# leimao/Voice-Converter-CycleGAN

Measured on NVIDIA H100. Metric: CycleGAN-VC train steps/sec @ batch 256x[24,128] MCEP, higher is better.
Workload: dtype f16f8 (forward / data gradient: fp16 MMA + two e4m3 cross-term MMAs = 2 MMA units per product; weight gradient: fp16 MMA alone, 1 unit; f32 accumulate)

## Files before the change

### voice-converter-cyclegan_b200/csrc/geom.h

```cpp
#pragma once
#include "kernels.cuh"
#include <string.h>
#include <vector>

static inline void same_pad(int n, int k, int s, int& before, int& out) {
  out = (n + s - 1) / s;
  int total = (out - 1) * s + k - n; if (total < 0) total = 0;
  before = total / 2;
}

static inline GatherGeom fwd_geom(int B, int H, int W, int kh, int kw, int sh, int sw) {
  GatherGeom g; memset(&g, 0, sizeof g);
  int ph, pw, Ho, Wo; same_pad(H, kh, sh, ph, Ho); same_pad(W, kw, sw, pw, Wo);
  g.B = B; g.Hy = Ho; g.Wx = Wo; g.Hs = H; g.Ws = W; g.sy = sh; g.sx = sw;
  g.Hd = Ho; g.Wd = Wo; g.dsy = 1; g.dsx = 1; g.doy = 0; g.dox = 0;
  g.ntaps = 0;
  for (int i = 0; i < kh; ++i) for (int j = 0; j < kw; ++j) {
    g.oy[g.ntaps] = (short)(i - ph); g.ox[g.ntaps] = (short)(j - pw); g.widx[g.ntaps] = (short)(i * kw + j); g.ntaps++;
  }
  return g;
}

static inline bool divisible(int v, int s) { return ((v % s) + s) % s == 0; }

static inline std::vector<GatherGeom> dgrad_geoms(int B, int H, int W, int kh, int kw, int sh, int sw) {
  std::vector<GatherGeom> out;
  int ph, pw, Ho, Wo; same_pad(H, kh, sh, ph, Ho); same_pad(W, kw, sw, pw, Wo);
  for (int py = 0; py < sh; ++py) for (int px = 0; px < sw; ++px) {
    GatherGeom g; memset(&g, 0, sizeof g);
    g.B = B; g.Hy = (H - py + sh - 1) / sh; g.Wx = (W - px + sw - 1) / sw;
    if (g.Hy <= 0 || g.Wx <= 0) continue;
    g.Hs = Ho; g.Ws = Wo; g.sy = 1; g.sx = 1;
    g.Hd = H; g.Wd = W; g.dsy = sh; g.dsx = sw; g.doy = py; g.dox = px;
    g.ntaps = 0;
    for (int i = 0; i < kh; ++i) for (int j = 0; j < kw; ++j) {
      if (!divisible(py + ph - i, sh) || !divisible(px + pw - j, sw)) continue;
      g.oy[g.ntaps] = (short)((py + ph - i) / sh); g.ox[g.ntaps] = (short)((px + pw - j) / sw);
      g.widx[g.ntaps] = (short)(i * kw + j); g.ntaps++;
    }
    out.push_back(g);
  }
  return out;
}
```

### voice-converter-cyclegan_b200/csrc/kernels.cuh

```cuda
#pragma once
#include <cuda_runtime.h>
#include <cuda_bf16.h>
#include <cuda_fp16.h>
#include <cuda_fp8.h>
#include <stdint.h>

#define CGVC_Q_ACT_SHI 1.0f
#define CGVC_Q_ACT_SLO 4096.0f
#define CGVC_Q_W_SHI 8.0f
#define CGVC_Q_W_SLO 32768.0f
#define CGVC_Q_ACC_SHIFT 15
#ifdef __CUDACC__
__device__ __forceinline__ uint32_t cgvc_e4m3x4(float a, float b, float c, float d) {
  const uint32_t lo = (uint32_t)__nv_cvt_float2_to_fp8x2(make_float2(a, b), __NV_SATFINITE, __NV_E4M3);
  const uint32_t hi = (uint32_t)__nv_cvt_float2_to_fp8x2(make_float2(c, d), __NV_SATFINITE, __NV_E4M3);
  return lo | (hi << 16);
}
__device__ __forceinline__ void cgvc_quant4(const float (&v)[4], float s_hi, float s_lo, uint2& q16, uint32_t& q8hi, uint32_t& q8lo) {
  const __half2 h01 = __floats2half2_rn(v[0], v[1]), h23 = __floats2half2_rn(v[2], v[3]);
  const float2 f01 = __half22float2(h01), f23 = __half22float2(h23);
  q16.x = *reinterpret_cast<const uint32_t*>(&h01); q16.y = *reinterpret_cast<const uint32_t*>(&h23);
  q8hi = cgvc_e4m3x4(f01.x * s_hi, f01.y * s_hi, f23.x * s_hi, f23.y * s_hi);
  q8lo = cgvc_e4m3x4((v[0] - f01.x) * s_lo, (v[1] - f01.y) * s_lo, (v[2] - f23.x) * s_lo, (v[3] - f23.y) * s_lo);
}
#endif

extern unsigned long long g_cgvc_launches;

#define CGVC_NUM_SMS 132

#define CGVC_MAX_TAPS 18

struct GatherGeom {
  int B, Hy, Wx;
  int Hs, Ws;
  int sy, sx;
  int ntaps;
  int Hd, Wd, dsy, dsx, doy, dox;
  short oy[CGVC_MAX_TAPS], ox[CGVC_MAX_TAPS], widx[CGVC_MAX_TAPS];
};

struct PackGeom { const long long* off; int n; int div; int max_len; };
#ifdef __CUDACC__
__device__ __forceinline__ int pack_find(const long long* __restrict__ off, int n, long long f) {
  int lo = 0, hi = n;
  while (hi - lo > 1) { const int mid = (lo + hi) >> 1; if (__ldg(off + mid) <= f) lo = mid; else hi = mid; }
  return lo;
}
#endif

struct GemmOperands {
  const float* src; int s_ld; int s_coff; int C;
  const float* w; long long w_ts; int w_cs; int w_ns;
  int N;
  float* dst; int d_ld; int d_coff;
  const float* bias;
  int accumulate;
};

cudaError_t launch_gg_simt(const GatherGeom& g, const GemmOperands& op, cudaStream_t st);
cudaError_t launch_gg_simt_packed(const GatherGeom& g, const GemmOperands& op, const PackGeom& pk, cudaStream_t st);
cudaError_t launch_wgrad_simt(const GatherGeom& g, const float* src, int s_ld, int s_coff, int C,
                              const float* grad, int g_ld, int g_coff, int N,
                              float* dw, long long w_ts, int w_cs, int w_ns, cudaStream_t st);
cudaError_t launch_colsum(const float* grad, long long rows, int g_ld, int g_coff, int N, float* db, cudaStream_t st);

struct PostParams {
  const float* p; int ldp; int Cc;
  int B, R, C, sh;
  const float *beta_a, *gamma_a, *beta_g, *gamma_g;
  int has_in, has_gate;
  const float* resid;
  float* y;
  float* stats;
  __nv_bfloat16 *y_hi, *y_lo;
  float* scratch;
  int qmode;
  PackGeom seg; long long seg_rows;
};
cudaError_t launch_post_fwd(const PostParams& pp, cudaStream_t st);

struct PostBwdParams {
  const float* dy1; const float* dy2;
  const float* p; int ldp; int Cc;
// ... 62 lines not shown
```

### voice-converter-cyclegan_b200/csrc/tc_gemm.cu

```cuda
#include "tc_gemm.cuh"
#include "geom.h"
#include "kernels.cuh"
#include "wgmma.cuh"

#include <cuda.h>
#include <stdint.h>
#include <stdio.h>

namespace {

typedef CUresult (*EncodeTiledFn)(CUtensorMap*, CUtensorMapDataType, cuuint32_t, void*, const cuuint64_t*, const cuuint64_t*,
                                  const cuuint32_t*, const cuuint32_t*, CUtensorMapInterleave, CUtensorMapSwizzle,
                                  CUtensorMapL2promotion, CUtensorMapFloatOOBfill);
EncodeTiledFn get_encoder() {
  static EncodeTiledFn fn = nullptr;
  if (!fn) {
    void* p = nullptr; cudaDriverEntryPointQueryResult q;
    if (cudaGetDriverEntryPoint("cuTensorMapEncodeTiled", &p, cudaEnableDefault, &q) == cudaSuccess && q == cudaDriverEntryPointSuccess)
      fn = (EncodeTiledFn)p;
  }
  return fn;
}
bool make_tmap3(CUtensorMap* m, const void* base, uint64_t d0, uint64_t d1, uint64_t d2, uint32_t b1) {
  EncodeTiledFn enc = get_encoder();
// ... 65 lines not shown
__device__ __forceinline__ void mbar_arrive(uint64_t* bar) {
  asm volatile("mbarrier.arrive.shared::cta.b64 _, [%0];" ::"r"(smem_u32(bar)) : "memory");
}
__device__ __forceinline__ void consumer_bar() { asm volatile("bar.sync 3, 256;" ::: "memory"); }
__device__ __forceinline__ void st_shared16(uint32_t addr, uint4 v) {
  asm volatile("st.shared.v4.b32 [%0], {%1, %2, %3, %4};" ::"r"(addr), "r"(v.x), "r"(v.y), "r"(v.z), "r"(v.w) : "memory");
}
__device__ __forceinline__ uint4 e4m3x8_to_f16x8(uint2 v) {
  uint32_t w[4];
#pragma unroll
  for (int i = 0; i < 4; ++i) {
    const uint32_t src = (i < 2 ? v.x : v.y) >> (16 * (i & 1));
    const __half2_raw h = __nv_cvt_fp8x2_to_halfraw2((__nv_fp8x2_storage_t)(src & 0xFFFFu), __NV_E4M3);
    w[i] = (uint32_t)h.x | ((uint32_t)h.y << 16);
  }
  return make_uint4(w[0], w[1], w[2], w[3]);
}

struct FastDiv { uint32_t mul, shr, d; };
__host__ inline FastDiv make_fastdiv(uint32_t d) {
  FastDiv f; f.d = d;
  uint32_t l = 0; while ((1ull << l) < d) ++l;
  f.mul = (uint32_t)(((1ull << 32) * ((1ull << l) - d)) / d + 1);
  f.shr = l;
  return f;
}
__device__ __forceinline__ uint32_t fdiv(uint32_t n, const FastDiv& f) { return (uint32_t)(((uint64_t)__umulhi(n, f.mul) + n) >> f.shr); }

__device__ __forceinline__ uint32_t sw128(int r, int c) { return (uint32_t)((r >> 3) * 1024 + (r & 7) * 128 + ((c ^ (r & 7)) << 4)); }

struct TcNTParams {
  GatherGeom g;
  const __nv_bfloat16 *a_hi, *a_lo; int a_ld; int C;
  const __nv_bfloat16 *b_hi, *b_lo; int Nw;
  int N;
  int n_tiles;
  int debug;
  float* dst; int d_ld; const float* bias; int accumulate;
  int perm; int Cc;
  int R;
  const float *gamma_a, *beta_a, *gamma_g, *beta_g;
  float* stats;
  const float* resid;
  float* y; __nv_bfloat16 *y_hi, *y_lo;
  int C_out;
  const float* bp; int bp_ld;
  __nv_bfloat16 *dp_hi, *dp_lo; int dp_ld;
  float *dbeta_a, *dgamma_a, *dbeta_g, *dgamma_g;
  CUtensorMap tm_b_hi, tm_b_lo;
  const uint8_t *a8_hi, *a8_lo;
  CUtensorMap tm_b8_hi, tm_b8_lo;
  uint8_t* y8;
  PackGeom pk;
};

struct TcTNParams {
  GatherGeom g;
  const __nv_bfloat16 *x_hi, *x_lo; int x_ld; int C;
  const __nv_bfloat16 *g_hi, *g_lo; int g_ld; int N;
  float* dw_a; float* dw_g; int n_split;
  int ksplit;
  FastDiv div_hw, div_w;
  CUtensorMap tm_g_hi, tm_g_lo;
  const uint8_t *x8_hi, *x8_lo;
  const uint8_t *g8_hi, *g8_lo;
  int w16;
  int fold_n;
};

__device__ __forceinline__ float* tn_dst(float* base, int slab, int C, int c, int ncols, int col, int fold_n) {
  if (fold_n) { const int t = col / fold_n; return base + ((long long)t * C + c) * fold_n + (col - t * fold_n); }
  return base + ((long long)slab * C + c) * ncols + col;
}

constexpr int kProducerThreads = 128;


template <int BN, int NPL>
struct NTCfg {
  static constexpr int A_PLANE = 128 * 128;
  static constexpr int B_PLANE = BN * 128;
  static constexpr int PLANES = NPL == 2 ? 2 : 1;
  static constexpr int STAGE = PLANES * (A_PLANE + B_PLANE);
  static constexpr int STAGES = (192 * 1024) / STAGE;
  static constexpr int SMEM = STAGES * STAGE + 1024;
  static_assert(STAGES * STAGE >= 128 * BN * 4, "the finished fp32 tile is staged over the pipeline stages");
};

template <int BN>
__device__ __forceinline__ int acc_off(int r, int n) { return r * BN + (n & ~31) + ((((n >> 2) & 7) ^ (r & 7)) << 2) + (n & 3); }
template <int BN>
__device__ __forceinline__ void acc_ld32(const float* acc, int r, int col, uint32_t (&v)[32]) {
#pragma unroll
  for (int c = 0; c < 8; ++c) {
    const float4 x = *reinterpret_cast<const float4*>(acc + r * BN + col + ((c ^ (r & 7)) << 2));
    v[4 * c] = __float_as_uint(x.x); v[4 * c + 1] = __float_as_uint(x.y); v[4 * c + 2] = __float_as_uint(x.z); v[4 * c + 3] = __float_as_uint(x.w);
  }
}

__device__ __forceinline__ float warp_colsum32(float (&t)[32], int lane) {
#pragma unroll
  for (int o = 16, n = 32; o >= 1; o >>= 1, n >>= 1) {
    const bool up = (lane & o) != 0;
#pragma unroll
    for (int i = 0; i < n / 2; ++i) {
      float send = up ? t[i] : t[i + n / 2];
      float keep = up ? t[i + n / 2] : t[i];
      t[i] = keep + __shfl_xor_sync(0xffffffffu, send, o);
    }
  }
  return t[0];
}
__device__ __forceinline__ void epi_bar(int id) { asm volatile("bar.sync %0, 128;" ::"r"(id) : "memory"); }

__device__ __forceinline__ float sample_sum(float v, float (*xch)[32], int q, int lane, int spw, int barid) {
  if (spw == 1) return v;
  epi_bar(barid);
  xch[q][lane] = v;
  epi_bar(barid);
  const int q0 = (q / spw) * spw;
  float r = 0.f;
  for (int w = 0; w < spw; ++w) r += xch[q0 + w][lane];
  return r;
}
__device__ __forceinline__ void bc4(const float* p, float (&v)[4]) { const float4 x = *reinterpret_cast<const float4*>(p); v[0] = x.x; v[1] = x.y; v[2] = x.z; v[3] = x.w; }
__device__ __forceinline__ float fast_sigmoid(float x) { return __fdividef(1.f, 1.f + __expf(-x)); }
__device__ __forceinline__ void chunk_norm_coeffs(const float (&v)[32], const float* __restrict__ gamma, const float* __restrict__ beta,
                                                  int ch, int R, float (*xch)[32], float* bc, int q, int lane, int spw, int barid, float& mean, float& rstd) {
  float t[32];
// ... 111 lines not shown
    rows_out(stg, y, lane, [&](int rr, int w0, float4 val) {
      if (mq + rr < M) *reinterpret_cast<float4*>(yf + ((mq + rr) * rs + ro) * C + ch + w0) = val;
    });
  float hl[32];
#pragma unroll
  for (int k = 0; k < 16; ++k) {
    __nv_bfloat162 hh = __floats2bfloat162_rn(y[2 * k], y[2 * k + 1]);
    float2 f = __bfloat1622float2(hh);
    __nv_bfloat162 ll = __floats2bfloat162_rn(y[2 * k] - f.x, y[2 * k + 1] - f.y);
    hl[k] = __uint_as_float(*reinterpret_cast<uint32_t*>(&hh)); hl[16 + k] = __uint_as_float(*reinterpret_cast<uint32_t*>(&ll));
  }
  rows_out(stg, hl, lane, [&](int rr, int w0, float4 val) {
    __nv_bfloat16* plane = (w0 < 16) ? yhi : ylo;
    if (mq + rr < M) *reinterpret_cast<float4*>(plane + ((mq + rr) * rs + ro) * C + ch + 2 * (w0 & 15)) = val;
  });
}
__device__ __forceinline__ void hwrite_yq(float* stg, const float (&y)[32], float* yf, __nv_bfloat16* q16, uint8_t* q8,
                                          long long mq, long long M, int C, int ch, int lane, int rs = 1, int ro = 0) {
  if (yf)
    rows_out(stg, y, lane, [&](int rr, int w0, float4 val) {
      if (mq + rr < M) *reinterpret_cast<float4*>(yf + ((mq + rr) * rs + ro) * C + ch + w0) = val;
    });
  float w[32];
#pragma unroll
  for (int k = 0; k < 8; ++k) {
    const float v[4] = {y[4 * k], y[4 * k + 1], y[4 * k + 2], y[4 * k + 3]};
    uint2 h; uint32_t b_hi, b_lo;
    cgvc_quant4(v, CGVC_Q_ACT_SHI, CGVC_Q_ACT_SLO, h, b_hi, b_lo);
    w[2 * k] = __uint_as_float(h.x); w[2 * k + 1] = __uint_as_float(h.y);
    w[16 + k] = __uint_as_float(b_hi); w[24 + k] = __uint_as_float(b_lo);
  }
  rows_out(stg, w, lane, [&](int rr, int w0, float4 val) {
    if (mq + rr >= M) return;
    const long long r = (mq + rr) * rs + ro;
    uint8_t* dst;
    if (w0 < 16) dst = reinterpret_cast<uint8_t*>(q16) + (r * C + ch + 2 * w0) * 2;
    else if (w0 < 24) dst = q8 + r * C + ch + 4 * (w0 - 16);
    else dst = q8 + M * rs * C + r * C + ch + 4 * (w0 - 24);
    *reinterpret_cast<float4*>(dst) = val;
  });
}

template <int BN, int NPL, int EPI>
__device__ __forceinline__ void nt_tile_epilogue(const TcNTParams& p, const long long M, const int HW, const long long m0, const int n0,
                                                 const int q, const int lane, float* stg, float** rowp, float* bc, float (*epi_xch)[32],
                                                 const float* acc, const int grp = 0, const int ngrp = 1) {
  const GatherGeom& g = p.g;
  const int barid = 1 + grp;
  const int arow = q * 32 + lane;
  const long long mq = m0 + q * 32;
  const long long m = mq + lane;
  float* drow = nullptr;
  if (m < M && p.dst) {
    int b = (int)(m / HW); int rem = (int)(m - (long long)b * HW);
    int y = rem / g.Wx; int x = rem - y * g.Wx;
    long long dr = ((long long)(b * g.Hd + y * g.dsy + g.doy) * g.Wd + x * g.dsx + g.dox);
    drow = p.dst + dr * p.d_ld;
  }
  __syncwarp();
  rowp[lane] = drow;
  __syncwarp();
  {
    const int spw = p.R >> 5;
    const long long sample = mq / p.R;
    const bool stat_writer = (q % spw) == 0 && mq < M && p.stats != nullptr;
    if (EPI == 1) {
      const int ch0 = n0 >> 1;
#pragma unroll 1
      for (int cb = grp; cb < 4; cb += ngrp) {
        const int ch = ch0 + cb * 32;
        float va[32], vg[32];
        { uint32_t u[32]; acc_ld32<BN>(acc, arow, (cb * 32), u);
#pragma unroll
          for (int k = 0; k < 32; k += 4) { float4 bb = *reinterpret_cast<const float4*>(p.bias + n0 + cb * 32 + k);
            va[k] = __uint_as_float(u[k]) + bb.x; va[k + 1] = __uint_as_float(u[k + 1]) + bb.y; va[k + 2] = __uint_as_float(u[k + 2]) + bb.z; va[k + 3] = __uint_as_float(u[k + 3]) + bb.w; } }
        { uint32_t u[32]; acc_ld32<BN>(acc, arow, (128 + cb * 32), u);
#pragma unroll
          for (int k = 0; k < 32; k += 4) { float4 bb = *reinterpret_cast<const float4*>(p.bias + n0 + 128 + cb * 32 + k);
            vg[k] = __uint_as_float(u[k]) + bb.x; vg[k + 1] = __uint_as_float(u[k + 1]) + bb.y; vg[k + 2] = __uint_as_float(u[k + 2]) + bb.z; vg[k + 3] = __uint_as_float(u[k + 3]) + bb.w; } }
        if (p.dst) {
          hwrite_rows_f32(stg, va, rowp, ch, lane);
          hwrite_rows_f32(stg, vg, rowp, p.Cc + ch, lane);
        }
        float mean_a, rstd_a, mean_g, rstd_g;
        chunk_norm_coeffs(va, p.gamma_a, p.beta_a, ch, p.R, epi_xch, bc, q, lane, spw, barid, mean_a, rstd_a);
        chunk_norm_coeffs(vg, p.gamma_g, p.beta_g, ch, p.R, epi_xch, bc + 64, q, lane, spw, barid, mean_g, rstd_g);
        if (stat_writer) {
          float* st = p.stats + sample * 4 * p.C_out + ch + lane;
          st[0] = mean_a; st[p.C_out] = rstd_a; st[2 * p.C_out] = mean_g; st[3 * p.C_out] = rstd_g;
        }
#pragma unroll
        for (int k = 0; k < 32; k += 4) {
          float4 sa = *reinterpret_cast<const float4*>(bc + k), oa = *reinterpret_cast<const float4*>(bc + 32 + k);
          float4 sg = *reinterpret_cast<const float4*>(bc + 64 + k), og = *reinterpret_cast<const float4*>(bc + 96 + k);
          va[k]     = fmaf(va[k],     sa.x, oa.x) * fast_sigmoid(fmaf(vg[k],     sg.x, og.x));
          va[k + 1] = fmaf(va[k + 1], sa.y, oa.y) * fast_sigmoid(fmaf(vg[k + 1], sg.y, og.y));
          va[k + 2] = fmaf(va[k + 2], sa.z, oa.z) * fast_sigmoid(fmaf(vg[k + 2], sg.z, og.z));
          va[k + 3] = fmaf(va[k + 3], sa.w, oa.w) * fast_sigmoid(fmaf(vg[k + 3], sg.w, og.w));
        }
        if (NPL == 3) hwrite_yq(stg, va, p.y, p.y_hi, p.y8, mq, M, p.C_out, ch, lane);
        else hwrite_y(stg, va, p.y, p.y_hi, p.y_lo, mq, M, p.C_out, ch, lane);
      }
    } else if (EPI == 5) {
      const int Ch = p.C_out;
      const int ch0 = n0 >> 2;
#pragma unroll 1
      for (int cb = grp; cb < 2; cb += ngrp) {
        const int ch = ch0 + cb * 32;
// ... 202 lines not shown
          wgmma_e4m3<BN>(d, make_desc(sA + 64 + k * 32, 16, 1024), make_desc64(sB + k * 32), 1);
        }
      } else if constexpr (KIND == MMA_F16) {
#pragma unroll
        for (int k = 0; k < 4; ++k)
          wgmma_f16<BN, 0, 0>(d, make_desc(sA + k * 32, 16, 1024), make_desc(sB + k * 32, 16, 1024), 1);
      } else {
#pragma unroll
        for (int k = 0; k < 4; ++k) {
          const uint64_t a_hi = make_desc(sA + k * 32, 16, 1024), b_hi = make_desc(sB + k * 32, 16, 1024);
          wgmma_bf16<BN, 0, 0>(d, a_hi, b_hi, 1);
          if constexpr (KIND == MMA_BF16X3) {
            const uint64_t a_lo = make_desc(sA + Cfg::A_PLANE + k * 32, 16, 1024), b_lo = make_desc(sB + Cfg::B_PLANE + k * 32, 16, 1024);
            wgmma_bf16<BN, 0, 0>(d, a_hi, b_lo, 1);
            wgmma_bf16<BN, 0, 0>(d, a_lo, b_hi, 1);
          }
        }
      }
    } else {
#pragma unroll
      for (int k = 0; k < 4; ++k) {
        const uint64_t a0 = make_desc(sA + k * 2048, 8192, 1024), b0 = make_desc(sB + k * 2048, 8192, 1024);
        const uint64_t a1 = make_desc(sA + Cfg::A_PLANE + k * 2048, 8192, 1024), b1 = make_desc(sB + Cfg::B_PLANE + k * 2048, 8192, 1024);
        if constexpr (KIND == MMA_F16_CROSS) {
          wgmma_f16<BN, 1, 1>(d, a0, b1, 1);
          wgmma_f16<BN, 1, 1>(d, a1, b0, 1);
        } else if constexpr (KIND == MMA_F16) {
          wgmma_f16<BN, 1, 1>(d, a0, b0, 1);
        } else {
          wgmma_bf16<BN, 1, 1>(d, a0, b0, 1);
          if constexpr (KIND == MMA_BF16X3) {
            wgmma_bf16<BN, 1, 1>(d, a0, b1, 1);
            wgmma_bf16<BN, 1, 1>(d, a1, b0, 1);
          }
        }
      }
    }
    wgmma_commit();
    wgmma_wait<1>();
    fence_acc(d);
    if (prev >= 0 && lane == 0) mbar_arrive(&empty_bar[prev]);
    prev = stage;
    if (++stage == Cfg::STAGES) { stage = 0; phase ^= 1; }
  }
}
template <int N>
__device__ __forceinline__ void rescale_acc(float (&d)[N], float scale) {
  wgmma_wait<0>();
  fence_acc(d);
#pragma unroll
  for (int i = 0; i < N; ++i) d[i] *= scale;
}

template <int BN>
__device__ __forceinline__ void nt_store_fragments(const TcNTParams& p, const float (&d)[BN / 2], const long long M, const int HW,
                                                   const long long m0, const int n0, const int r, const int c) {
  const GatherGeom& g = p.g;
  float* rowp[2];
#pragma unroll
  for (int h = 0; h < 2; ++h) {
    const long long m = m0 + r + 8 * h;
    rowp[h] = nullptr;
    if (m < M && p.dst) {
      int b = (int)(m / HW); int rem = (int)(m - (long long)b * HW);
      int y = rem / g.Wx; int x = rem - y * g.Wx;
      rowp[h] = p.dst + ((long long)(b * g.Hd + y * g.dsy + g.doy) * g.Wd + x * g.dsx + g.dox) * p.d_ld;
    }
  }
  const bool vec = (p.d_ld & 1) == 0;
#pragma unroll
  for (int j = 0; j < BN / 8; ++j) {
    const int cb = j >> 2;
    const int n = (p.perm == 2 ? (cb >> 2) * p.Cc + ((cb >> 1) & 1) * (p.Cc >> 1) + (n0 >> 2) + (cb & 1) * 32
                   : p.perm    ? ((cb < 4) ? (n0 >> 1) + cb * 32 : p.Cc + (n0 >> 1) + (cb - 4) * 32) : n0 + cb * 32) + ((8 * j) & 31) + c;
    if (n >= p.N) continue;
    float2 bb = make_float2(0.f, 0.f);
    if (p.bias) bb = *reinterpret_cast<const float2*>(p.bias + n0 + 8 * j + c);
#pragma unroll
    for (int h = 0; h < 2; ++h) {
      float* rp = rowp[h];
      if (rp == nullptr) continue;
      float v0 = d[4 * j + 2 * h], v1 = d[4 * j + 2 * h + 1];
      if (p.bias) { v0 += bb.x; v1 += bb.y; }
      if (vec && n + 2 <= p.N) {
        if (p.accumulate)
          asm volatile("red.global.add.v2.f32 [%0], {%1, %2};" ::"l"(rp + n), "f"(v0), "f"(v1) : "memory");
        else
          *reinterpret_cast<float2*>(rp + n) = make_float2(v0, v1);
      } else {
        if (p.accumulate) atomicAdd(rp + n, v0); else rp[n] = v0;
        if (n + 1 < p.N) { if (p.accumulate) atomicAdd(rp + n + 1, v1); else rp[n + 1] = v1; }
      }
    }
  }
}

constexpr int kNTThreads = 384;

template <int BN, int NPL, int EPI, bool PK = false>
__global__ void __launch_bounds__(kNTThreads, 1)
tc_gg_nt_kernel(const __grid_constant__ TcNTParams p) {
  static_assert(!PK || EPI == 0, "packed rows never take the fused epilogues (they need whole equal-length samples per tile)");
  using Cfg = NTCfg<BN, NPL>;
  __shared__ float epi_xch[2][4][32];
  __shared__ __align__(16) float epi_bc[8][(EPI == 3 || EPI == 4) ? 384 : 128];
  __shared__ __align__(16) float epi_stage[8][32 * 16];
  __shared__ float* epi_rowp[8][32];
  constexpr int S = Cfg::STAGES;
  extern __shared__ uint8_t smem_raw[];
  __shared__ __align__(8) uint64_t full_bar[S], empty_bar[S], acc_free_bar;

  const uint32_t smem_base = (smem_u32(smem_raw) + 1023u) & ~1023u;
  const int warp = threadIdx.x >> 5, lane = threadIdx.x & 31;
  const GatherGeom& g = p.g;
  const long long M = (long long)g.B * g.Hy * g.Wx;
  const int HW = g.Hy * g.Wx;
  const int cchunks = p.C >> 6;
  const int kb_pass = g.ntaps * cchunks;
  const int num_kb = NPL == 3 ? 2 * kb_pass : kb_pass;
  const int m_tiles = (int)((M + 127) / 128);
  const int n_tiles = p.n_tiles;
  const int num_tiles = m_tiles * n_tiles;

  if (threadIdx.x == 0) {
    for (int s = 0; s < S; ++s) { mbar_init(&full_bar[s], kProducerThreads + 1); mbar_init(&empty_bar[s], 8); }
    mbar_init(&acc_free_bar, 8);
    fence_barrier_init();
    tma_prefetch_desc(&p.tm_b_hi);
    if (NPL == 2) tma_prefetch_desc(&p.tm_b_lo);
    if (NPL == 3) { tma_prefetch_desc(&p.tm_b8_hi); tma_prefetch_desc(&p.tm_b8_lo); }
  }
  __syncthreads();

  if (warp < 4) {
    const int t = threadIdx.x;
    const int chunk = t & 7, rsub = t >> 3;
    int stage = 0; uint32_t phase = 0;
    int it = 0;
    for (int tile = blockIdx.x; tile < num_tiles; tile += gridDim.x, ++it) {
      const long long m0 = (long long)(tile % m_tiles) * 128;
      const int n0 = (tile / m_tiles) * BN;
      if (EPI != 0 && it > 0) mbar_wait(&acc_free_bar, (uint32_t)(it - 1) & 1u);
      int rb[8], ry[8], rx[8];
#pragma unroll
      for (int i = 0; i < 8; ++i) {
        long long m = m0 + rsub + 16 * i;
        if (m < M) {
          if constexpr (PK) {
            const int dout = p.pk.div * g.sx;
            const int u = pack_find(p.pk.off, p.pk.n, m * dout);
            const long long o0 = __ldg(p.pk.off + u), o1 = __ldg(p.pk.off + u + 1);
            rb[i] = (int)(o0 / p.pk.div); ry[i] = (int)((o1 - o0) / p.pk.div); rx[i] = (int)(m - o0 / dout) * g.sx;
          } else {
            int b = (int)(m / HW); int rem = (int)(m - (long long)b * HW);
            int y = rem / g.Wx; int x = rem - y * g.Wx;
            rb[i] = b; ry[i] = y * g.sy; rx[i] = x * g.sx;
          }
        } else { rb[i] = -1; ry[i] = 0; rx[i] = 0; }
      }
      for (int pass = 0; pass < (NPL == 3 ? 2 : 1); ++pass)
      for (int tap = 0; tap < g.ntaps; ++tap) {
        long long aoff[8];
#pragma unroll
        for (int i = 0; i < 8; ++i) {
          const int cofs = NPL == 3 && pass == 0 ? (chunk & 3) * 16 : chunk * 8;
          if constexpr (PK) {
            const int xx = rx[i] + g.ox[tap];
            aoff[i] = rb[i] >= 0 && xx >= 0 && xx < ry[i] ? (long long)(rb[i] + xx) * p.a_ld + cofs : -1;
          } else {
            int yy = ry[i] + g.oy[tap], xx = rx[i] + g.ox[tap];
            bool ok = rb[i] >= 0 && yy >= 0 && yy < g.Hs && xx >= 0 && xx < g.Ws;
            aoff[i] = ok ? ((long long)(rb[i] * g.Hs + yy) * g.Ws + xx) * p.a_ld + cofs : -1;
          }
        }
        for (int cc = 0; cc < cchunks; ++cc) {
          const int c0 = cc << 6;
          mbar_wait(&empty_bar[stage], phase ^ 1);
          const uint32_t sA = smem_base + stage * Cfg::STAGE;
          const uint32_t sB = sA + Cfg::PLANES * Cfg::A_PLANE;
          if (t == 0) {
            mbar_expect_tx(&full_bar[stage], Cfg::PLANES * Cfg::B_PLANE);
            if (NPL == 3) {
              if (pass == 0) {
                tma_load3(sB, &p.tm_b8_hi, c0, n0, g.widx[tap], &full_bar[stage]);
                tma_load3(sB + Cfg::B_PLANE / 2, &p.tm_b8_lo, c0, n0, g.widx[tap], &full_bar[stage]);
              } else {
                tma_load3(sB, &p.tm_b_hi, c0, n0, g.widx[tap], &full_bar[stage]);
              }
            } else {
              tma_load3(sB, &p.tm_b_hi, c0, n0, g.widx[tap], &full_bar[stage]);
              if (NPL == 2) tma_load3(sB + Cfg::B_PLANE, &p.tm_b_lo, c0, n0, g.widx[tap], &full_bar[stage]);
            }
          }
          if (!(p.debug & 4)) {
#pragma unroll
            for (int i = 0; i < 8; ++i) {
              const int r = rsub + 16 * i;
              const uint32_t so = sw128(r, chunk);
              const bool ok = aoff[i] >= 0;
              const long long off = ok ? aoff[i] + c0 : 0;
              if (NPL == 3) {
                if (pass == 0)
                  cp_async16(sA + so, (chunk < 4 ? p.a8_hi : p.a8_lo) + off, ok ? 16u : 0u);
                else
                  cp_async16(sA + so, p.a_hi + off, ok ? 16u : 0u);
              } else {
                cp_async16(sA + so, p.a_hi + off, ok ? 16u : 0u);
                if (NPL == 2) cp_async16(sA + Cfg::A_PLANE + so, p.a_lo + off, ok ? 16u : 0u);
              }
            }
          }
          cp_async_arrive_noinc(&full_bar[stage]);
          if (++stage == S) { stage = 0; phase ^= 1; }
        }
      }
    }
  } else {
    const int cw = warp - 4;
    const int wg = cw >> 2;
    const int tw = threadIdx.x - 128 * (wg + 1);
    float* acc_s = reinterpret_cast<float*>(smem_raw + (smem_base - smem_u32(smem_raw)));
    int stage = 0; uint32_t phase = 0;
    for (int tile = blockIdx.x; tile < num_tiles; tile += gridDim.x) {
      const long long m0 = (long long)(tile % m_tiles) * 128;
      const int n0 = (tile / m_tiles) * BN;
      float d[BN / 2];
#pragma unroll
      for (int i = 0; i < BN / 2; ++i) d[i] = 0.f;
      int prev = -1;
      if constexpr (NPL == 3) {
        consume_stages<BN, MMA_E4M3_CROSS, 0, Cfg>(d, kb_pass, stage, phase, prev, full_bar, empty_bar, smem_base, wg, lane);
        rescale_acc(d, 1.f / (float)(1 << CGVC_Q_ACC_SHIFT));
        consume_stages<BN, MMA_F16, 0, Cfg>(d, kb_pass, stage, phase, prev, full_bar, empty_bar, smem_base, wg, lane);
      } else {
        consume_stages<BN, NPL == 2 ? MMA_BF16X3 : MMA_BF16, 0, Cfg>(d, num_kb, stage, phase, prev, full_bar, empty_bar, smem_base, wg, lane);
      }
      wgmma_wait<0>();
      fence_acc(d);
      if (lane == 0) mbar_arrive(&empty_bar[prev]);
      const int r0 = wg * 64 + (tw >> 5) * 16 + ((tw & 31) >> 2), c0 = 2 * (tw & 3);
      if constexpr (EPI == 0) {
        if (!(p.debug & 3)) nt_store_fragments<BN>(p, d, M, HW, m0, n0, r0, c0);
      } else {
        consumer_bar();
        if (!(p.debug & 2)) {
#pragma unroll
          for (int j = 0; j < BN / 8; ++j) {
            *reinterpret_cast<float2*>(acc_s + acc_off<BN>(r0, 8 * j + c0)) = make_float2(d[4 * j], d[4 * j + 1]);
            *reinterpret_cast<float2*>(acc_s + acc_off<BN>(r0 + 8, 8 * j + c0)) = make_float2(d[4 * j + 2], d[4 * j + 3]);
          }
        }
        consumer_bar();
        nt_tile_epilogue<BN, NPL, EPI>(p, M, HW, m0, n0, cw & 3, lane, epi_stage[cw], epi_rowp[cw], epi_bc[cw], epi_xch[wg], acc_s, wg, 2);
        fence_proxy_async();
        __syncwarp();
        if (lane == 0) mbar_arrive(&acc_free_bar);
      }
    }
  }
}

#define CGVC_Q_WGRAD_SHIFT 12
template <int NPL, int W16>
struct TNCfg {
  static constexpr int A_PLANE = 64 * 256;
  static constexpr int B_PLANE = 64 * 512;
  static constexpr int PLANES = (NPL == 1 || W16) ? 1 : 2;
  static constexpr int STAGE = PLANES * (A_PLANE + B_PLANE);
  static constexpr int STAGES = (192 * 1024) / STAGE;
  static constexpr int SMEM = STAGES * STAGE + 1024;
};

template <int NPL, int W16>
__global__ void __launch_bounds__(kNTThreads, 1)
tc_gg_tn_kernel(const __grid_constant__ TcTNParams p) {
  static_assert(W16 == 0 || NPL == 3, "the fp16-only weight gradient is a form of CGVC_PREC_F16F8");
  using Cfg = TNCfg<NPL, W16>;
  constexpr int S = Cfg::STAGES;
  constexpr int BN = 256;
  extern __shared__ uint8_t smem_raw[];
  __shared__ __align__(8) uint64_t full_bar[S], empty_bar[S];

  const uint32_t smem_base = (smem_u32(smem_raw) + 1023u) & ~1023u;
  const int warp = threadIdx.x >> 5, lane = threadIdx.x & 31;
  const GatherGeom& g = p.g;
  const long long M = (long long)g.B * g.Hy * g.Wx;
  const int HW = g.Hy * g.Wx;
  const int n_tiles = (p.g_ld + BN - 1) / BN, c_tiles = (p.x_ld + 127) / 128;
  const int num_items = n_tiles * c_tiles * g.ntaps * p.ksplit;
  constexpr int pass0 = (NPL == 3 && !W16) ? 0 : 1;
  long long chunk_rows = (M + p.ksplit - 1) / p.ksplit;
  chunk_rows = (chunk_rows + 63) / 64 * 64;

  struct Item { int n0, c0, tap; long long mbeg, mend; int num_kb; };
  auto decode = [&](int item) -> Item {
// ... 279 lines not shown
    const int cig = (lane & 3) * 8;
    const int col = warp * 8 + (lane >> 2);
    const int co = co0 + col;
    if (co < J.cout && ci0 + cig < J.cin_q) {
      float va[4], vb[4];
#pragma unroll
      for (int k = 0; k < 4; ++k) { va[k] = tile[cig + k][col]; vb[k] = tile[cig + 4 + k][col]; }
      const int nrow = perm_row(J.perm, co, J.cout, J.noff);
      const long long o = ((long long)tap * J.nt_n + nrow) * J.cin_q + ci0 + cig;
      uint2 ha, hb; uint32_t a_hi, a_lo, b_hi, b_lo;
      cgvc_quant4(va, CGVC_Q_W_SHI, CGVC_Q_W_SLO, ha, a_hi, a_lo);
      cgvc_quant4(vb, CGVC_Q_W_SHI, CGVC_Q_W_SLO, hb, b_hi, b_lo);
      *reinterpret_cast<uint4*>(J.q16 + o) = make_uint4(ha.x, ha.y, hb.x, hb.y);
      *reinterpret_cast<uint2*>(J.q8hi + o) = make_uint2(a_hi, b_hi);
      *reinterpret_cast<uint2*>(J.q8lo + o) = make_uint2(a_lo, b_lo);
    }
  }
  if (tap == 0 && tci == 0 && tco == 0 && J.b_off >= 0)
    for (int i = t; i < J.cout; i += 256) J.bias[perm_row(J.perm, i, J.cout, J.noff)] = params[J.b_off + i];
}

template <class K>
cudaError_t set_smem(K kernel, int bytes) {
  static std::vector<const void*> done;
  const void* key = (const void*)kernel;
  for (const void* d : done) if (d == key) return cudaSuccess;
  cudaError_t e = cudaFuncSetAttribute(kernel, cudaFuncAttributeMaxDynamicSharedMemorySize, bytes);
  if (e == cudaSuccess) done.push_back(key);
  return e;
}

struct ProfRec { cudaEvent_t a, b; double flops; int cls; long long M; int N, K; };
int g_tc_debug = 0;
int g_tc_prep_batched = 1;
bool g_prof_on = false;
std::vector<ProfRec> g_prof;
void prof_begin(cudaStream_t st, double flops, int cls, long long M = 0, int N = 0, int K = 0) {
  if (!g_prof_on) return;
  ProfRec r; r.flops = flops; r.cls = cls; r.M = M; r.N = N; r.K = K;
  cudaEventCreate(&r.a); cudaEventCreate(&r.b);
  cudaEventRecord(r.a, st);
  g_prof.push_back(r);
}
void prof_end(cudaStream_t st) { if (g_prof_on && !g_prof.empty()) cudaEventRecord(g_prof.back().b, st); }

inline int tile_rows(int n_real, int n_padded) { return (n_padded % 256 == 0) ? 256 : (n_real <= 32 ? 32 : 128); }

int num_sms() {
  static int n = 0;
  if (!n) { int dev = 0; cudaGetDevice(&dev); cudaDeviceGetAttribute(&n, cudaDevAttrMultiProcessorCount, dev); }
  return n;
}

cudaError_t launch_nt(TcNTParams p, int precision, cudaStream_t st, int epi) {
  const long long M = (long long)p.g.B * p.g.Hy * p.g.Wx;
  if (M == 0) return cudaSuccess;
  const bool x3 = precision == 1;
  if (p.g.ntaps == 0) return cudaErrorInvalidValue;
  const int bn = tile_rows(p.N, p.Nw);
  p.n_tiles = bn == 32 ? 1 : p.Nw / bn;
  const long long tiles = ((M + 127) / 128) * p.n_tiles;
  dim3 grid((unsigned)(tiles < num_sms() ? tiles : num_sms()));
  cudaError_t e;
  ++g_cgvc_launches;
  p.debug = g_tc_debug;
  prof_begin(st, 2.0 * (double)M * p.N * p.g.ntaps * p.C, (epi == 1 || epi == 2 || epi == 5) ? 2 : 0, M, p.N, p.g.ntaps * p.C);
#define LAUNCH_NT(BN_, NPL_, EPI_, ...)                                                                        \
  do {                                                                                                         \
    e = set_smem(tc_gg_nt_kernel<BN_, NPL_, EPI_, ##__VA_ARGS__>, NTCfg<BN_, NPL_>::SMEM);                     \
    if (e != cudaSuccess) return e;                                                                            \
    tc_gg_nt_kernel<BN_, NPL_, EPI_, ##__VA_ARGS__><<<grid, kNTThreads, NTCfg<BN_, NPL_>::SMEM, st>>>(p);      \
  } while (0)
  if (epi != 0 && bn != 256) return cudaErrorInvalidValue;
  if (p.pk.off) {
    if (epi != 0 || p.g.B != 1 || p.g.Hy != 1) return cudaErrorInvalidValue;
    const int npl = precision == 3 ? 3 : x3 ? 2 : 1;
    if (bn == 256)      { if (npl == 3) LAUNCH_NT(256, 3, 0, true); else if (npl == 2) LAUNCH_NT(256, 2, 0, true); else LAUNCH_NT(256, 1, 0, true); }
    else if (bn == 128) { if (npl == 3) LAUNCH_NT(128, 3, 0, true); else if (npl == 2) LAUNCH_NT(128, 2, 0, true); else LAUNCH_NT(128, 1, 0, true); }
    else                { if (npl == 3) LAUNCH_NT(32, 3, 0, true);  else if (npl == 2) LAUNCH_NT(32, 2, 0, true);  else LAUNCH_NT(32, 1, 0, true); }
  }
  else if (precision == 3) {
    if (epi == 1)       LAUNCH_NT(256, 3, 1);
    else if (epi == 2)  LAUNCH_NT(256, 3, 2);
    else if (epi == 5)  LAUNCH_NT(256, 3, 5);
    else if (epi != 0)  return cudaErrorInvalidValue;
    else if (bn == 256) LAUNCH_NT(256, 3, 0);
    else if (bn == 128) LAUNCH_NT(128, 3, 0);
    else                LAUNCH_NT(32, 3, 0);
  }
  else if (epi == 1)  { if (x3) LAUNCH_NT(256, 2, 1); else LAUNCH_NT(256, 1, 1); }
  else if (epi == 2)  { if (x3) LAUNCH_NT(256, 2, 2); else LAUNCH_NT(256, 1, 2); }
  else if (epi == 3)  { if (x3) LAUNCH_NT(256, 2, 3); else LAUNCH_NT(256, 1, 3); }
  else if (epi == 4)  { if (x3) LAUNCH_NT(256, 2, 4); else LAUNCH_NT(256, 1, 4); }
  else if (epi == 5)  { if (x3) LAUNCH_NT(256, 2, 5); else LAUNCH_NT(256, 1, 5); }
  else if (bn == 256) { if (x3) LAUNCH_NT(256, 2, 0); else LAUNCH_NT(256, 1, 0); }
  else if (bn == 128) { if (x3) LAUNCH_NT(128, 2, 0); else LAUNCH_NT(128, 1, 0); }
  else                { if (x3) LAUNCH_NT(32, 2, 0);  else LAUNCH_NT(32, 1, 0); }
#undef LAUNCH_NT
  prof_end(st);
  return cudaGetLastError();
}

cudaError_t launch_tn(TcTNParams p, int precision, cudaStream_t st) {
  const long long M = (long long)p.g.B * p.g.Hy * p.g.Wx;
  if (M == 0) return cudaSuccess;
  if (M >= (1ll << 31)) return cudaErrorInvalidValue;
  const int tiles = ((p.g_ld + 255) / 256) * ((p.x_ld + 127) / 128) * p.g.ntaps;
  const int nsm = num_sms();
  long long maxsplit = M / 1024; if (maxsplit < 1) maxsplit = 1; if (maxsplit > 32) maxsplit = 32;
  int ksplit = 1; double best = 0.0;
  for (int ks = 1; ks <= (int)maxsplit; ++ks) {
    long long items = (long long)tiles * ks;
    double eff = (double)items / (double)(((items + nsm - 1) / nsm) * nsm);
    if (items < nsm) eff *= 0.5;
    if (eff > best + 0.02) { best = eff; ksplit = ks; }
  }
  p.ksplit = ksplit;
  p.div_hw = make_fastdiv((uint32_t)(p.g.Hy * p.g.Wx)); p.div_w = make_fastdiv((uint32_t)p.g.Wx);
  const long long items = (long long)tiles * ksplit;
  dim3 grid((unsigned)(items < nsm ? items : nsm));
  cudaError_t e;
  ++g_cgvc_launches;
  prof_begin(st, 2.0 * (double)M * p.N * p.g.ntaps * p.C, 1, M, p.N, p.g.ntaps * p.C);
#define LAUNCH_TN(NPL_, W16_)                                                                     \
  do {                                                                                            \
    e = set_smem(tc_gg_tn_kernel<NPL_, W16_>, TNCfg<NPL_, W16_>::SMEM);                           \
    if (e != cudaSuccess) return e;                                                               \
// ... 216 lines not shown
      L.wq16 = p; p += rnd(wq_elems(L) * 2);
      L.wq8hi = (uint8_t*)p; p += rnd(wq_elems(L)); L.wq8lo = (uint8_t*)p; p += rnd(wq_elems(L));
      if (w.quant_bwd) {
        L.wdq16 = p; p += rnd(wdq_elems(L) * 2);
        L.wdq8hi = (uint8_t*)p; p += rnd(wdq_elems(L)); L.wdq8lo = (uint8_t*)p; p += rnd(wdq_elems(L));
      }
      if (!make_layer_maps_q(L)) return (int)cudaErrorInvalidValue;
    }
  }
  w.job_first.clear(); w.job_ka.clear();
  if (w.quant) {
    std::vector<PrepJob> jobs;
    int blocks = 0;
    for (TcLayer& L : w.layers) {
      if (!L.wq16) continue;
      for (int br = 0; br < (L.gated ? 2 : 1); ++br) {
        PrepJob J; memset(&J, 0, sizeof J);
        J.w_off = (long long)(br ? L.kg : L.ka); J.b_off = L.fold ? -1 : (long long)(br ? L.bg : L.ba);
        J.taps = L.kh * L.kw; J.cin = L.cin; J.cout = L.cout; J.nt_n = nt_n(L); J.cin_q = cin_q(L); J.cin_n = cin_n(L); J.nt_q = nt_q(L);
        J.noff = br ? L.cout : 0; J.perm = layer_perm(L); J.fold_n = L.fold ? L.cout / L.fold : 0;
        J.q16 = (__half*)L.wq16; J.q8hi = L.wq8hi; J.q8lo = L.wq8lo;
        J.dq16 = (__half*)L.wdq16; J.dq8hi = L.wdq8hi; J.dq8lo = L.wdq8lo;
        J.bias = L.bias;
        J.tiles_ci = (L.cin + 31) / 32; J.tiles_co = (L.cout + 63) / 64;
        J.first_block = blocks;
        blocks += J.taps * J.tiles_ci * J.tiles_co;
        jobs.push_back(J); w.job_first.push_back(J.first_block); w.job_ka.push_back(L.ka);
      }
    }
    w.job_first.push_back(blocks);
    if (!jobs.empty()) {
      err = cudaMalloc(&w.prep_jobs, jobs.size() * sizeof(PrepJob));
      if (err != cudaSuccess) return (int)err;
      err = cudaMemcpy(w.prep_jobs, jobs.data(), jobs.size() * sizeof(PrepJob), cudaMemcpyHostToDevice);
      if (err != cudaSuccess) return (int)err;
    }
  }
  w.ready = false;
  return 0;
}

static cudaError_t tc_init_kernels() {
  cudaError_t e;
#define INIT_NT(BN_, NPL_, EPI_) if ((e = set_smem(tc_gg_nt_kernel<BN_, NPL_, EPI_>, NTCfg<BN_, NPL_>::SMEM)) != cudaSuccess) return e;
  INIT_NT(256, 2, 0) INIT_NT(256, 1, 0) INIT_NT(128, 2, 0) INIT_NT(128, 1, 0) INIT_NT(32, 2, 0) INIT_NT(32, 1, 0)
  INIT_NT(256, 2, 1) INIT_NT(256, 1, 1) INIT_NT(256, 2, 2) INIT_NT(256, 1, 2)
  INIT_NT(256, 2, 3) INIT_NT(256, 1, 3) INIT_NT(256, 2, 4) INIT_NT(256, 1, 4) INIT_NT(256, 2, 5) INIT_NT(256, 1, 5)
  INIT_NT(256, 3, 0) INIT_NT(128, 3, 0) INIT_NT(32, 3, 0) INIT_NT(256, 3, 1) INIT_NT(256, 3, 2) INIT_NT(256, 3, 5)
#undef INIT_NT
#define INIT_NT_PK(BN_, NPL_) if ((e = set_smem(tc_gg_nt_kernel<BN_, NPL_, 0, true>, NTCfg<BN_, NPL_>::SMEM)) != cudaSuccess) return e;
  INIT_NT_PK(256, 1) INIT_NT_PK(256, 2) INIT_NT_PK(256, 3) INIT_NT_PK(128, 1) INIT_NT_PK(128, 2) INIT_NT_PK(128, 3)
  INIT_NT_PK(32, 1) INIT_NT_PK(32, 2) INIT_NT_PK(32, 3)
#undef INIT_NT_PK
#define INIT_TN(NPL_, W16_) if ((e = set_smem(tc_gg_tn_kernel<NPL_, W16_>, TNCfg<NPL_, W16_>::SMEM)) != cudaSuccess) return e;
  INIT_TN(3, 1) INIT_TN(3, 0) INIT_TN(2, 0) INIT_TN(1, 0)
#undef INIT_TN
  return cudaSuccess;
}

void tc_free(TcWeights& w) {
  if (w.pool) cudaFree(w.pool);
  if (w.prep_jobs) cudaFree(w.prep_jobs);
  w.pool = nullptr; w.prep_jobs = nullptr; w.ready = false;
}

static int refresh_jobs(TcWeights& w, const float* params, int j0, int j1, cudaStream_t st) {
  if (j1 <= j0) return 0;
  const int b0 = w.job_first[j0], nb = w.job_first[j1] - b0;
  ++g_cgvc_launches;
  prep_weights_q_all_kernel<<<(unsigned)nb, 256, 0, st>>>(params, (const PrepJob*)w.prep_jobs, j0, j1, b0);
  return (int)cudaGetLastError();
}

int tc_refresh_weights(TcWeights& w, const float* params, cudaStream_t st) {
  if (!w.pool) return 0;
  const bool batched = g_tc_prep_batched && w.prep_jobs;
  for (TcLayer& L : w.layers) {
    if (batched && L.wq16) continue;
    int r = refresh_layer(L, params + L.ka, params + L.kg, params + L.ba, params + L.bg, st);
    if (r != 0) return r;
  }
  if (batched) { int r = refresh_jobs(w, params, 0, (int)w.job_ka.size(), st); if (r != 0) return r; }
  w.ready = true;
  return 0;
}

int tc_refresh_weights_range(TcWeights& w, const float* params, size_t begin, size_t end, cudaStream_t st) {
  if (!w.pool) return 0;
  const bool batched = g_tc_prep_batched && w.prep_jobs;
  for (TcLayer& L : w.layers) {
    if (L.ka < begin || L.ka >= end) continue;
    if (batched && L.wq16) continue;
    int r = refresh_layer(L, params + L.ka, params + L.kg, params + L.ba, params + L.bg, st);
    if (r != 0) return r;
  }
  if (batched) {
    const int nj = (int)w.job_ka.size();
    int j = 0;
    while (j < nj) {
      if (w.job_ka[j] < begin || w.job_ka[j] >= end) { ++j; continue; }
      int k = j; while (k < nj && w.job_ka[k] >= begin && w.job_ka[k] < end) ++k;
      int r = refresh_jobs(w, params, j, k, st); if (r != 0) return r;
      j = k;
    }
  }
  return 0;
// ... 137 lines not shown
```

Baseline: 9.559.

## Walk implicit-GEMM rows position-major and skip padded taps per tile

Adds a host-built position-major row table for the dense NT conv kernel. Output positions are sorted by how many kernel taps land inside the image, and rows are laid out batch-fastest, so each 128-row tile shares nearly the same valid-tap mask. The producer and consumer then skip the K-blocks of taps that fall entirely in zero padding. The path is used only when the table fits in 512 positions and enough K-blocks are removed. In exchange it adds a 2KB parameter table, a scattered output-row mapping, serpentine tile ordering, and more kernel template instantiations.

```diff
diff --git a/voice-converter-cyclegan_b200/csrc/geom.h b/voice-converter-cyclegan_b200/csrc/geom.h
--- a/voice-converter-cyclegan_b200/csrc/geom.h
+++ b/voice-converter-cyclegan_b200/csrc/geom.h
@@ -23,6 +23,27 @@
 
 static inline bool divisible(int v, int s) { return ((v % s) + s) % s == 0; }
 
+static inline uint32_t pos_taps(const GatherGeom& g, int y, int x) {
+  uint32_t m = 0;
+  for (int t = 0; t < g.ntaps; ++t) {
+    const int yy = y * g.sy + g.oy[t], xx = x * g.sx + g.ox[t];
+    if (yy >= 0 && yy < g.Hs && xx >= 0 && xx < g.Ws) m |= 1u << t;
+  }
+  return m;
+}
+
+static inline bool pm_table(const GatherGeom& g, uint32_t* tab) {
+  const int hw = g.Hy * g.Wx;
+  if (hw > CGVC_PM_MAX_POS) return false;
+  int n = 0;
+  for (int c = g.ntaps; c >= 0; --c)
+    for (int pos = 0; pos < hw; ++pos) {
+      const uint32_t m = pos_taps(g, pos / g.Wx, pos % g.Wx);
+      if (__builtin_popcount(m) == c) tab[n++] = (uint32_t)pos | (m << 10);
+    }
+  return true;
+}
+
 static inline std::vector<GatherGeom> dgrad_geoms(int B, int H, int W, int kh, int kw, int sh, int sw) {
   std::vector<GatherGeom> out;
   int ph, pw, Ho, Wo; same_pad(H, kh, sh, ph, Ho); same_pad(W, kw, sw, pw, Wo);
diff --git a/voice-converter-cyclegan_b200/csrc/kernels.cuh b/voice-converter-cyclegan_b200/csrc/kernels.cuh
--- a/voice-converter-cyclegan_b200/csrc/kernels.cuh
+++ b/voice-converter-cyclegan_b200/csrc/kernels.cuh
@@ -30,6 +30,7 @@
 #define CGVC_NUM_SMS 132
 
 #define CGVC_MAX_TAPS 18
+#define CGVC_PM_MAX_POS 512
 
 struct GatherGeom {
   int B, Hy, Wx;
diff --git a/voice-converter-cyclegan_b200/csrc/tc_gemm.cu b/voice-converter-cyclegan_b200/csrc/tc_gemm.cu
--- a/voice-converter-cyclegan_b200/csrc/tc_gemm.cu
+++ b/voice-converter-cyclegan_b200/csrc/tc_gemm.cu
@@ -141,6 +141,8 @@
   CUtensorMap tm_b8_hi, tm_b8_lo;
   uint8_t* y8;
   PackGeom pk;
+  int pm;
+  uint32_t pm_tab[CGVC_PM_MAX_POS];
 };
 
 struct TcTNParams {
@@ -164,6 +166,28 @@
 
 constexpr int kProducerThreads = 128;
 
+template <bool PM>
+__device__ __forceinline__ void nt_row(const TcNTParams& p, long long m, int HW, int& b, int& y, int& x) {
+  const GatherGeom& g = p.g;
+  int pos;
+  if constexpr (PM) { const int r = (int)(m / g.B); b = (int)(m - (long long)r * g.B); pos = (int)(p.pm_tab[r] & 1023u); }
+  else { b = (int)(m / HW); pos = (int)(m - (long long)b * HW); }
+  y = pos / g.Wx; x = pos - y * g.Wx;
+}
+template <bool PM>
+__device__ __forceinline__ uint32_t nt_tile_taps(const TcNTParams& p, long long m0, long long M) {
+  const uint32_t all = (1u << p.g.ntaps) - 1u;
+  if constexpr (!PM) return all;
+  const int r1 = (int)(((m0 + 128 < M ? m0 + 128 : M) - 1) / p.g.B);
+  uint32_t taps = 0;
+  for (int r = (int)(m0 / p.g.B); r <= r1 && taps != all; ++r) taps |= p.pm_tab[r] >> 10;
+  return taps ? taps : 1u;
+}
+template <bool PM>
+__device__ __forceinline__ int nt_tile(int it) {
+  return it * (int)gridDim.x + ((PM && (it & 1)) ? (int)(gridDim.x - 1 - blockIdx.x) : (int)blockIdx.x);
+}
+
 
 template <int BN, int NPL>
 struct NTCfg {
@@ -381,8 +405,7 @@
   const long long m = mq + lane;
   float* drow = nullptr;
   if (m < M && p.dst) {
-    int b = (int)(m / HW); int rem = (int)(m - (long long)b * HW);
-    int y = rem / g.Wx; int x = rem - y * g.Wx;
+    int b, y, x; nt_row<false>(p, m, HW, b, y, x);
     long long dr = ((long long)(b * g.Hd + y * g.dsy + g.doy) * g.Wd + x * g.dsx + g.dox);
     drow = p.dst + dr * p.d_ld;
   }
@@ -691,7 +714,7 @@
   for (int i = 0; i < N; ++i) d[i] *= scale;
 }
 
-template <int BN>
+template <int BN, bool PM>
 __device__ __forceinline__ void nt_store_fragments(const TcNTParams& p, const float (&d)[BN / 2], const long long M, const int HW,
                                                    const long long m0, const int n0, const int r, const int c) {
   const GatherGeom& g = p.g;
@@ -701,8 +724,7 @@
     const long long m = m0 + r + 8 * h;
     rowp[h] = nullptr;
     if (m < M && p.dst) {
-      int b = (int)(m / HW); int rem = (int)(m - (long long)b * HW);
-      int y = rem / g.Wx; int x = rem - y * g.Wx;
+      int b, y, x; nt_row<PM>(p, m, HW, b, y, x);
       rowp[h] = p.dst + ((long long)(b * g.Hd + y * g.dsy + g.doy) * g.Wd + x * g.dsx + g.dox) * p.d_ld;
     }
   }
@@ -736,10 +758,11 @@
 
 constexpr int kNTThreads = 384;
 
-template <int BN, int NPL, int EPI, bool PK = false>
+template <int BN, int NPL, int EPI, bool PK = false, bool PM = false>
 __global__ void __launch_bounds__(kNTThreads, 1)
 tc_gg_nt_kernel(const __grid_constant__ TcNTParams p) {
   static_assert(!PK || EPI == 0, "packed rows never take the fused epilogues (they need whole equal-length samples per tile)");
+  static_assert(!PM || (EPI == 0 && !PK), "the position-major walk is a form of the plain dense epilogue");
   using Cfg = NTCfg<BN, NPL>;
   __shared__ float epi_xch[2][4][32];
   __shared__ __align__(16) float epi_bc[8][(EPI == 3 || EPI == 4) ? 384 : 128];
@@ -755,8 +778,7 @@
   const long long M = (long long)g.B * g.Hy * g.Wx;
   const int HW = g.Hy * g.Wx;
   const int cchunks = p.C >> 6;
-  const int kb_pass = g.ntaps * cchunks;
-  const int num_kb = NPL == 3 ? 2 * kb_pass : kb_pass;
+  const int kb_all = g.ntaps * cchunks;
   const int m_tiles = (int)((M + 127) / 128);
   const int n_tiles = p.n_tiles;
   const int num_tiles = m_tiles * n_tiles;
@@ -776,10 +798,11 @@
     const int chunk = t & 7, rsub = t >> 3;
     int stage = 0; uint32_t phase = 0;
     int it = 0;
-    for (int tile = blockIdx.x; tile < num_tiles; tile += gridDim.x, ++it) {
+    for (int tile = nt_tile<PM>(0); tile < num_tiles; ++it, tile = PM ? nt_tile<PM>(it) : tile + (int)gridDim.x) {
       const long long m0 = (long long)(tile % m_tiles) * 128;
       const int n0 = (tile / m_tiles) * BN;
       if (EPI != 0 && it > 0) mbar_wait(&acc_free_bar, (uint32_t)(it - 1) & 1u);
+      const uint32_t taps = nt_tile_taps<PM>(p, m0, M);
       int rb[8], ry[8], rx[8];
 #pragma unroll
       for (int i = 0; i < 8; ++i) {
@@ -791,14 +814,14 @@
             const long long o0 = __ldg(p.pk.off + u), o1 = __ldg(p.pk.off + u + 1);
             rb[i] = (int)(o0 / p.pk.div); ry[i] = (int)((o1 - o0) / p.pk.div); rx[i] = (int)(m - o0 / dout) * g.sx;
           } else {
-            int b = (int)(m / HW); int rem = (int)(m - (long long)b * HW);
-            int y = rem / g.Wx; int x = rem - y * g.Wx;
+            int b, y, x; nt_row<PM>(p, m, HW, b, y, x);
             rb[i] = b; ry[i] = y * g.sy; rx[i] = x * g.sx;
           }
         } else { rb[i] = -1; ry[i] = 0; rx[i] = 0; }
       }
       for (int pass = 0; pass < (NPL == 3 ? 2 : 1); ++pass)
       for (int tap = 0; tap < g.ntaps; ++tap) {
+        if (PM && !((taps >> tap) & 1u)) continue;
         long long aoff[8];
 #pragma unroll
         for (int i = 0; i < 8; ++i) {
@@ -860,9 +883,10 @@
     const int tw = threadIdx.x - 128 * (wg + 1);
     float* acc_s = reinterpret_cast<float*>(smem_raw + (smem_base - smem_u32(smem_raw)));
     int stage = 0; uint32_t phase = 0;
-    for (int tile = blockIdx.x; tile < num_tiles; tile += gridDim.x) {
+    for (int it = 0, tile = nt_tile<PM>(0); tile < num_tiles; ++it, tile = PM ? nt_tile<PM>(it) : tile + (int)gridDim.x) {
       const long long m0 = (long long)(tile % m_tiles) * 128;
       const int n0 = (tile / m_tiles) * BN;
+      const int kb_pass = PM ? __popc(nt_tile_taps<PM>(p, m0, M)) * cchunks : kb_all;
       float d[BN / 2];
 #pragma unroll
       for (int i = 0; i < BN / 2; ++i) d[i] = 0.f;
@@ -872,14 +896,14 @@
         rescale_acc(d, 1.f / (float)(1 << CGVC_Q_ACC_SHIFT));
         consume_stages<BN, MMA_F16, 0, Cfg>(d, kb_pass, stage, phase, prev, full_bar, empty_bar, smem_base, wg, lane);
       } else {
-        consume_stages<BN, NPL == 2 ? MMA_BF16X3 : MMA_BF16, 0, Cfg>(d, num_kb, stage, phase, prev, full_bar, empty_bar, smem_base, wg, lane);
+        consume_stages<BN, NPL == 2 ? MMA_BF16X3 : MMA_BF16, 0, Cfg>(d, kb_pass, stage, phase, prev, full_bar, empty_bar, smem_base, wg, lane);
       }
       wgmma_wait<0>();
       fence_acc(d);
       if (lane == 0) mbar_arrive(&empty_bar[prev]);
       const int r0 = wg * 64 + (tw >> 5) * 16 + ((tw & 31) >> 2), c0 = 2 * (tw & 3);
       if constexpr (EPI == 0) {
-        if (!(p.debug & 3)) nt_store_fragments<BN>(p, d, M, HW, m0, n0, r0, c0);
+        if (!(p.debug & 3)) nt_store_fragments<BN, PM>(p, d, M, HW, m0, n0, r0, c0);
       } else {
         consumer_bar();
         if (!(p.debug & 2)) {
@@ -1265,6 +1289,18 @@
   return n;
 }
 
+long long pm_kept_kb(const uint32_t* tab, int B, long long M, int ntaps) {
+  const uint32_t all = (1u << ntaps) - 1u;
+  long long kept = 0;
+  for (long long m0 = 0; m0 < M; m0 += 128) {
+    const int r1 = (int)(((m0 + 128 < M ? m0 + 128 : M) - 1) / B);
+    uint32_t taps = 0;
+    for (int r = (int)(m0 / B); r <= r1 && taps != all; ++r) taps |= tab[r] >> 10;
+    kept += taps ? __builtin_popcount(taps) : 1;
+  }
+  return kept;
+}
+
 cudaError_t launch_nt(TcNTParams p, int precision, cudaStream_t st, int epi) {
   const long long M = (long long)p.g.B * p.g.Hy * p.g.Wx;
   if (M == 0) return cudaSuccess;
@@ -1277,6 +1313,7 @@
   cudaError_t e;
   ++g_cgvc_launches;
   p.debug = g_tc_debug;
+  p.pm = (epi == 0 && !p.pk.off && p.g.Hy > 1 && pm_table(p.g, p.pm_tab) && pm_kept_kb(p.pm_tab, p.g.B, M, p.g.ntaps) * 8 <= ((M + 127) / 128) * p.g.ntaps * 7) ? 1 : 0;
   prof_begin(st, 2.0 * (double)M * p.N * p.g.ntaps * p.C, (epi == 1 || epi == 2 || epi == 5) ? 2 : 0, M, p.N, p.g.ntaps * p.C);
 #define LAUNCH_NT(BN_, NPL_, EPI_, ...)                                                                        \
   do {                                                                                                         \
@@ -1285,7 +1322,13 @@
     tc_gg_nt_kernel<BN_, NPL_, EPI_, ##__VA_ARGS__><<<grid, kNTThreads, NTCfg<BN_, NPL_>::SMEM, st>>>(p);      \
   } while (0)
   if (epi != 0 && bn != 256) return cudaErrorInvalidValue;
-  if (p.pk.off) {
+  if (p.pm) {
+    const int npl = precision == 3 ? 3 : x3 ? 2 : 1;
+    if (bn == 256)      { if (npl == 3) LAUNCH_NT(256, 3, 0, false, true); else if (npl == 2) LAUNCH_NT(256, 2, 0, false, true); else LAUNCH_NT(256, 1, 0, false, true); }
+    else if (bn == 128) { if (npl == 3) LAUNCH_NT(128, 3, 0, false, true); else if (npl == 2) LAUNCH_NT(128, 2, 0, false, true); else LAUNCH_NT(128, 1, 0, false, true); }
+    else                { if (npl == 3) LAUNCH_NT(32, 3, 0, false, true);  else if (npl == 2) LAUNCH_NT(32, 2, 0, false, true);  else LAUNCH_NT(32, 1, 0, false, true); }
+  }
+  else if (p.pk.off) {
     if (epi != 0 || p.g.B != 1 || p.g.Hy != 1) return cudaErrorInvalidValue;
     const int npl = precision == 3 ? 3 : x3 ? 2 : 1;
     if (bn == 256)      { if (npl == 3) LAUNCH_NT(256, 3, 0, true); else if (npl == 2) LAUNCH_NT(256, 2, 0, true); else LAUNCH_NT(256, 1, 0, true); }
@@ -1608,6 +1651,10 @@
   INIT_NT_PK(256, 1) INIT_NT_PK(256, 2) INIT_NT_PK(256, 3) INIT_NT_PK(128, 1) INIT_NT_PK(128, 2) INIT_NT_PK(128, 3)
   INIT_NT_PK(32, 1) INIT_NT_PK(32, 2) INIT_NT_PK(32, 3)
 #undef INIT_NT_PK
+#define INIT_NT_PM(BN_, NPL_) if ((e = set_smem(tc_gg_nt_kernel<BN_, NPL_, 0, false, true>, NTCfg<BN_, NPL_>::SMEM)) != cudaSuccess) return e;
+  INIT_NT_PM(256, 1) INIT_NT_PM(256, 2) INIT_NT_PM(256, 3) INIT_NT_PM(128, 1) INIT_NT_PM(128, 2) INIT_NT_PM(128, 3)
+  INIT_NT_PM(32, 1) INIT_NT_PM(32, 2) INIT_NT_PM(32, 3)
+#undef INIT_NT_PM
 #define INIT_TN(NPL_, W16_) if ((e = set_smem(tc_gg_tn_kernel<NPL_, W16_>, TNCfg<NPL_, W16_>::SMEM)) != cudaSuccess) return e;
   INIT_TN(3, 1) INIT_TN(3, 0) INIT_TN(2, 0) INIT_TN(1, 0)
 #undef INIT_TN
```

Result: faster. 9.806 (median of 6 runs) (+2.6%).
